# bayesiains/nflows

Hardware: NVIDIA H100
Metric: Flow.log_prob samples/sec, 10-layer RQ-NSF D=784 (higher is better)
Workload: dtype f32

## Files before the change

### nflows_b200/csrc/fused_spline.cuh

```cuda
#pragma once
#include "rq_spline.cuh"
#include "tc_common.cuh"

namespace nfk {
namespace tc {

template <int NB, bool TAILS>
struct FusedCfg {
    static constexpr int M = TAILS ? 3 * NB - 1 : 3 * NB + 1;
    static constexpr int MP = (M + 7) / 8 * 8;
    static constexpr int FPT = BN / (2 * MP);
    static constexpr int TF = 2 * FPT;
    static constexpr int TILE = TF * MP;
    static_assert(FPT >= 1, "unsupported bin count for the fused kernels");
};

struct SplineOut {
    const float* bias;
    const float* x;
    float* y;
    __half* y_hi;
    __half* y_lo;
    const int32_t* t_cols;
    int t_col0;
    float out_scale;
    int64_t ldx, ldy, lds;
    int d_t;
    int inverse;
    float inv_acc_scale;
    SplineParams sp;
};

template <int NB, bool TAILS>
__device__ __forceinline__ int stg_chunk(int r, int c) {
    constexpr int C = FusedCfg<NB, TAILS>::FPT * FusedCfg<NB, TAILS>::MP / 4;
    return c ^ ((0x6530 >> (4 * (r & 3))) & 7) ^ ((C % 8 == 0 && c >= C) ? 4 : 0);
}

template <int NB, bool TAILS, int N>
__device__ __forceinline__ void stage_sums(float* stg, const float (&sum)[N / 2], int wi, int lane) {
#pragma unroll
    for (int j = 0; j < N / 8; ++j)
#pragma unroll
        for (int h = 0; h < 2; ++h) {
            const int r = wi * 16 + (lane >> 2) + 8 * h, c = 2 * j + ((lane & 3) >> 1);
            *reinterpret_cast<float2*>(stg + r * BN + 4 * stg_chunk<NB, TAILS>(r, c) + 2 * (lane & 1)) =
                make_float2(sum[4 * j + 2 * h], sum[4 * j + 2 * h + 1]);
        }
}

template <int NB, bool TAILS>
struct SplineIn {
    float x[FusedCfg<NB, TAILS>::FPT];
    int col[FusedCfg<NB, TAILS>::FPT];
};
template <int NB, bool TAILS>
__device__ __forceinline__ SplineIn<NB, TAILS> spline_inputs(const SplineOut& o, int n, int64_t row, bool row_ok, int fh) {
    constexpr int FPT = FusedCfg<NB, TAILS>::FPT, TF = FusedCfg<NB, TAILS>::TF;
    const int j0 = n * TF + fh * FPT;
    SplineIn<NB, TAILS> in;
#pragma unroll
    for (int f = 0; f < FPT; ++f) {
        const bool ok = row_ok && (j0 + f < o.d_t);
        in.col[f] = !ok ? 0 : (o.t_cols ? __ldg(o.t_cols + j0 + f) : o.t_col0 + j0 + f);
        in.x[f] = ok ? o.x[row * o.ldx + in.col[f]] : 0.0f;
    }
    return in;
}

template <int NB, bool TAILS>
__device__ __forceinline__ void spline_tile(const SplineOut& o, const float* stg, int r, int n, int64_t row, bool row_ok, int fh,
                                            const SplineIn<NB, TAILS>& in, float& lad_row, int& flag) {
    using Cfg = FusedCfg<NB, TAILS>;
    constexpr int MP = Cfg::MP, FPT = Cfg::FPT, TF = Cfg::TF, TILE = Cfg::TILE, C = FPT * MP / 4;
    const int j0 = n * TF + fh * FPT;
    float v[FPT * MP];
    const float* b = o.bias + (int64_t)n * TILE + fh * FPT * MP;
#pragma unroll
    for (int i = 0; i < C; ++i) {
        const float4 s = *reinterpret_cast<const float4*>(stg + r * BN + 4 * stg_chunk<NB, TAILS>(r, fh * C + i));
        const float sv[4] = {s.x, s.y, s.z, s.w};
#pragma unroll
        for (int e = 0; e < 4; ++e) {
            const int c = 4 * i + e;
            v[c] = fmaf(sv[e], o.inv_acc_scale, (j0 + c / MP < o.d_t) ? __ldg(b + c) : 0.0f);
        }
    }
    float yy[FPT], ll[FPT];
    if (o.inverse) rqs_eval_lean<NB, TAILS, true, FPT, MP>(o.sp, in.x, v, yy, ll, flag);
    else rqs_eval_lean<NB, TAILS, false, FPT, MP>(o.sp, in.x, v, yy, ll, flag);
#pragma unroll
    for (int f = 0; f < FPT; ++f) {
        if (!(row_ok && j0 + f < o.d_t)) continue;
        lad_row += ll[f];
        if (o.y_hi) {
            __half hi, lo;
            split_f16(yy[f], o.out_scale, hi, lo, flag);
            o.y_hi[row * o.lds + in.col[f]] = hi;
            o.y_lo[row * o.lds + in.col[f]] = lo;
        } else {
            o.y[row * o.ldy + in.col[f]] = yy[f];
        }
    }
}

}
}
```

### nflows_b200/csrc/nfk_coupling_step_tc.cu

```cuda
#include <stdlib.h>
#include <string.h>

#include "fused_spline.cuh"

namespace nfk {
namespace tc {

constexpr int STEP_MAX_LAYERS = 9;
constexpr int STEP_MAX_HIDDEN = 256;
constexpr int STEP_DRAIN_TRUNK = 4;
constexpr int STEP_DRAIN_FINAL = 8;
constexpr int STEP_SLAB_BYTES = 2 * A_BYTES;
constexpr int STEP_R_BYTES = (STEP_MAX_HIDDEN / BK) * STEP_SLAB_BYTES;
constexpr int STEP_G0_STAGES = STEP_R_BYTES / STAGE_BYTES;
constexpr int STEP_S_OFF = STEP_R_BYTES;
constexpr int STEP_S_WG_BYTES = 32768;
constexpr int STEP_W_OFF = STEP_S_OFF + 2 * STEP_S_WG_BYTES;
constexpr int STEP_W_STAGES = 2;
constexpr int STEP_W_STAGE_BYTES = 2 * B_BYTES;
constexpr int STEP_BAR_OFF = STEP_W_OFF + STEP_W_STAGES * STEP_W_STAGE_BYTES;
constexpr int STEP_LAD_OFF = STEP_BAR_OFF + 256;
constexpr int STEP_SMEM_BYTES = STEP_LAD_OFF + 512 + 1024 ;
static_assert(64 * BN * 4 <= STEP_S_WG_BYTES && 4 * 2 * 64 * 64 <= STEP_S_WG_BYTES, "S");
static_assert(STEP_SMEM_BYTES <= 232448, "coupling-step kernel shared memory");
static_assert(STEP_MAX_HIDDEN / BK <= STEP_DRAIN_FINAL, "the final layer drains once (mma_final)");

constexpr int SL_RELU_OUT = 1;
constexpr int SL_ADD_SKIP = 2;
constexpr int SL_SAVE_SKIP = 4;
constexpr int SL_SPLIT_RELU = 8;

struct StepParams {
    const float* bias_trunk;
    float* skip_buf;
    int H, K0, num_layers;
    int layer_flags[STEP_MAX_LAYERS];
    float acc_scale[STEP_MAX_LAYERS], inv_acc_scale[STEP_MAX_LAYERS];
    float act_scale;
    __half* h_hi;
    __half* h_lo;
    int64_t ldh;
    SplineOut o;
    float* lad_accum;
    int32_t* flags;
    int64_t n_rows;
    int num_m_tiles, num_n_tiles;
};

__device__ __forceinline__ void put_pair(uint8_t* base, int slab_stride, int lo_off, int r, int col, float x0, float x1, float scale,
                                         float& amax) {
    x0 *= scale; x1 *= scale;
    amax = fmaxf(amax, fmaxf(fabsf(x0), fabsf(x1)));
    const __half2 h = __floats2half2_rn(x0, x1);
    const float2 hf = __half22float2(h);
    const __half2 l = __floats2half2_rn(x0 - hf.x, x1 - hf.y);
    const int k = col & 31;
    uint8_t* q = base + (col >> 5) * slab_stride + r * 64 + (((k >> 3) ^ ((r >> 1) & 3)) << 4) + (k & 7) * 2;
    *reinterpret_cast<__half2*>(q) = h;
    *reinterpret_cast<__half2*>(q + lo_off) = l;
}

__device__ __forceinline__ void consumers_sync() { asm volatile("bar.sync 3, 256;" ::: "memory"); }
constexpr int STEP_BAR_TURN = 4;
constexpr int STEP_BAR_LAD = 6;

template <int N, int MH>
__device__ __forceinline__ void mma_final(float (&acc)[MH][N / 2], Ring& r, int num_k, uint32_t a_res, int lane, int turn) {
    int prev = -1;
    for (int j = 0; j < num_k; ++j) {
        mbar_wait(r.full + 8 * r.stage, r.phase);
        if (turn >= 0 && j == num_k - 1) {
            __threadfence_block();
            pair_arrive(turn);
        }
        const uint32_t sw = r.base + r.stage * r.stage_bytes;
        const uint64_t w_hi = make_smem_desc(sw), w_lo = make_smem_desc(sw + B_BYTES);
        wgmma_fence();
#pragma unroll
        for (int m = 0; m < MH; ++m) {
            const uint32_t sa = a_res + (uint32_t)j * STEP_SLAB_BYTES + m * (A_BYTES / 2);
            const uint64_t a_hi = make_smem_desc(sa), a_lo = make_smem_desc(sa + A_BYTES);
#pragma unroll
            for (int kk = 0; kk < BK / 16; ++kk) {
                const uint64_t adv = (uint64_t)(kk * 2);
                wgmma_f16<N>(acc[m], a_lo + adv, w_hi + adv, (j | kk) != 0);
                wgmma_f16<N>(acc[m], a_hi + adv, w_lo + adv, 1);
            }
#pragma unroll
            for (int kk = 0; kk < BK / 16; ++kk) {
                const uint64_t adv = (uint64_t)(kk * 2);
                wgmma_f16<N>(acc[m], a_hi + adv, w_hi + adv, 1);
            }
        }
        wgmma_commit();
        if (prev >= 0) {
            wgmma_wait<1>();
            __syncwarp();
            if (lane == 0) mbar_arrive(r.empty + 8 * prev, MH);
        }
        prev = r.stage;
        r.advance();
    }
    wgmma_wait<0>();
    __syncwarp();
    if (lane == 0) mbar_arrive(r.empty + 8 * prev, MH);
}

template <int NB, bool TAILS>
__global__ void __launch_bounds__(THREADS, 1)
rq_coupling_step_kernel(const __grid_constant__ CUtensorMap map_a_hi, const __grid_constant__ CUtensorMap map_a_lo,
                        const __grid_constant__ CUtensorMap map_w0_hi, const __grid_constant__ CUtensorMap map_w0_lo,
                        const __grid_constant__ CUtensorMap map_wt_hi, const __grid_constant__ CUtensorMap map_wt_lo,
                        const __grid_constant__ CUtensorMap map_wf_hi, const __grid_constant__ CUtensorMap map_wf_lo,
                        const StepParams p) {
    constexpr int TILE = FusedCfg<NB, TAILS>::TILE;
    extern __shared__ uint8_t smem_raw[];
    const uint32_t smem_base = (smem_u32(smem_raw) + 1023u) & ~1023u;
    uint8_t* smem_gen = smem_raw + (smem_base - smem_u32(smem_raw));
    const uint32_t bars = smem_base + STEP_BAR_OFF;
    Ring ring0{smem_base, bars, bars + 8 * STEP_G0_STAGES, STEP_G0_STAGES, (uint32_t)STAGE_BYTES};
    Ring ring1{smem_base + STEP_W_OFF, bars + 64, bars + 64 + 8 * STEP_W_STAGES, STEP_W_STAGES, (uint32_t)STEP_W_STAGE_BYTES};
    const uint32_t bar_rfree = bars + 96;
    const int warp = threadIdx.x >> 5, lane = threadIdx.x & 31;
    const int H = p.H;
    const int num_k0 = (p.K0 + BK - 1) / BK, num_kh = H / BK;
    const int nch = (H + BN - 1) / BN;
    const bool trunk_only = p.h_hi != nullptr;

    if (threadIdx.x == 0) {
        for (int s = 0; s < STEP_G0_STAGES; ++s) { mbar_init(ring0.full + 8 * s, 1); mbar_init(ring0.empty + 8 * s, 8); }
        for (int s = 0; s < STEP_W_STAGES; ++s) { mbar_init(ring1.full + 8 * s, 1); mbar_init(ring1.empty + 8 * s, 8); }
        mbar_init(bar_rfree, 8);
        asm volatile("fence.mbarrier_init.release.cluster;" ::: "memory");
        prefetch_tmap(&map_a_hi); prefetch_tmap(&map_a_lo); prefetch_tmap(&map_w0_hi); prefetch_tmap(&map_w0_lo);
        prefetch_tmap(&map_wt_hi); prefetch_tmap(&map_wt_lo); prefetch_tmap(&map_wf_hi); prefetch_tmap(&map_wf_lo);
    }
    __syncthreads();

    if (warp < 4) {
        asm volatile("setmaxnreg.dec.sync.aligned.u32 40;" ::: "memory");
        if (warp == 0 && elect_one()) {
            uint32_t rphase = 0;
            for (int u = blockIdx.x; u < p.num_m_tiles; u += gridDim.x) {
                if (u != (int)blockIdx.x) { mbar_wait(bar_rfree, rphase); rphase ^= 1; }
                for (int c = 0; c < nch; ++c)
                    for (int ks = 0; ks < num_k0; ++ks) produce_slab(ring0, &map_a_hi, &map_a_lo, &map_w0_hi, &map_w0_lo, ks, u * BM, c * BN);
                for (int l = 1; l < p.num_layers; ++l)
                    for (int c = 0; c < nch; ++c)
                        for (int ks = 0; ks < num_kh; ++ks) produce_w_slab(ring1, &map_wt_hi, &map_wt_lo, ks, (l - 1) * H + c * BN);
                if (!trunk_only)
                    for (int n = 0; n < p.num_n_tiles; ++n)
                        for (int ks = 0; ks < num_kh; ++ks) produce_w_slab(ring1, &map_wf_hi, &map_wf_lo, ks, n * TILE, TILE);
            }
        }
        return;
    }
    asm volatile("setmaxnreg.inc.sync.aligned.u32 232;" ::: "memory");
    const int wg = (warp >> 2) - 1, wi = warp & 3, q = lane & 3;
    const int t = threadIdx.x - 128 * (1 + wg);
    const int r_loc = t >> 1, fh = t & 1;
    uint8_t* R = smem_gen;
    uint8_t* S = smem_gen + STEP_S_OFF + wg * STEP_S_WG_BYTES;
    float* stg = reinterpret_cast<float*>(S);
    float* skip = p.skip_buf + (size_t)blockIdx.x * BM * H;
    int flag = 0;
    for (int u = blockIdx.x; u < p.num_m_tiles; u += gridDim.x) {
        const int64_t m0 = (int64_t)u * BM;
        int rt[2];
        rt[0] = wg * 64 + wi * 16 + (lane >> 2);
        rt[1] = rt[0] + 8;
        for (int l = 0; l < p.num_layers; ++l) {
            const int lf = p.layer_flags[l];
            const bool to_global = trunk_only && l == p.num_layers - 1;
            const float as = p.acc_scale[l], ias = p.inv_acc_scale[l];
            float amax = 0.0f;
            for (int c = 0; c < nch; ++c) {
                const int cb = c * BN + 2 * q;
                float sum[64];
#pragma unroll
                for (int j = 0; j < 16; ++j) {
                    const int col = cb + 8 * j;
#pragma unroll
                    for (int e = 0; e < 2; ++e) {
                        const float b = col < H ? __ldg(p.bias_trunk + l * H + col + e) * as : 0.0f;
#pragma unroll
                        for (int h = 0; h < 2; ++h) {
                            const float sk = ((lf & SL_ADD_SKIP) && col < H) ? skip[rt[h] * H + col + e] : 0.0f;
                            sum[4 * j + 2 * h + e] = fmaf(sk, as, b);
                        }
                    }
                }
                if (l == 0) mma_tile(sum, ring0, num_k0, STEP_DRAIN_TRUNK, wg, lane);
                else mma_tile(sum, ring1, num_kh, STEP_DRAIN_TRUNK, wg, lane, smem_base);
#pragma unroll
                for (int i = 0; i < 64; ++i) {
                    float x = sum[i] * ias;
                    if (lf & SL_RELU_OUT) x = fmaxf(x, 0.0f);
                    sum[i] = x;
                }
                if (lf & SL_SAVE_SKIP) {
#pragma unroll
                    for (int j = 0; j < 16; ++j)
#pragma unroll
                        for (int h = 0; h < 2; ++h)
                            if (cb + 8 * j < H)
                                *reinterpret_cast<float2*>(skip + rt[h] * H + cb + 8 * j) = make_float2(sum[4 * j + 2 * h], sum[4 * j + 2 * h + 1]);
                }
                if (lf & SL_SPLIT_RELU) {
#pragma unroll
                    for (int i = 0; i < 64; ++i) sum[i] = fmaxf(sum[i], 0.0f);
                }
                if (to_global) {
#pragma unroll
                    for (int h = 0; h < 2; ++h) {
                        const int64_t row = m0 + rt[h];
                        if (row >= p.n_rows) continue;
                        float am = 0.0f;
#pragma unroll
                        for (int j = 0; j < 16; ++j) {
                            const int col = cb + 8 * j;
                            if (col >= H) continue;
                            const float x0 = sum[4 * j + 2 * h] * p.act_scale, x1 = sum[4 * j + 2 * h + 1] * p.act_scale;
                            am = fmaxf(am, fmaxf(fabsf(x0), fabsf(x1)));
                            const __half2 hh = __floats2half2_rn(x0, x1);
                            const float2 hf = __half22float2(hh);
                            *reinterpret_cast<__half2*>(p.h_hi + row * p.ldh + col) = hh;
                            *reinterpret_cast<__half2*>(p.h_lo + row * p.ldh + col) = __floats2half2_rn(x0 - hf.x, x1 - hf.y);
                        }
                        if (!(am <= 65000.0f)) flag |= 4;
                    }
                    continue;
                }
                const bool into_r = c == nch - 1;
                if (into_r) {
                    if (l == 0) consumers_sync();
                } else {
                    wg_sync(wg);
                }
#pragma unroll
                for (int h = 0; h < 2; ++h) {
                    float am = 0.0f;
#pragma unroll
                    for (int j = 0; j < 16; ++j) {
                        const int cc = 8 * j + 2 * q;
                        if (c * BN + cc >= H) continue;
                        if (into_r)
                            put_pair(R, STEP_SLAB_BYTES, A_BYTES, rt[h], c * BN + cc, sum[4 * j + 2 * h], sum[4 * j + 2 * h + 1], p.act_scale, am);
                        else
                            put_pair(S, 2 * A_BYTES / 2, A_BYTES / 2, rt[h] - wg * 64, cc, sum[4 * j + 2 * h], sum[4 * j + 2 * h + 1],
                                     p.act_scale, am);
                    }
                    if (m0 + rt[h] < p.n_rows) amax = fmaxf(amax, am);
                }
                if (into_r && nch > 1) {
                    wg_sync(wg);
                    for (int i = t; i < 4 * 2 * 256; i += 128) {
                        const int part = i >> 8, k = i & 255;
                        const uint4 v = reinterpret_cast<const uint4*>(S + part * 4096)[k];
                        reinterpret_cast<uint4*>(R + (part >> 1) * STEP_SLAB_BYTES + (part & 1) * A_BYTES + wg * 4096)[k] = v;
                    }
                }
            }
            if (!(amax <= 65000.0f)) flag |= 4;
            if (!to_global) {
                asm volatile("fence.proxy.async.shared::cta;" ::: "memory");
                wg_sync(wg);
            }
        }
        if (trunk_only) {
            __syncwarp();
            if (lane == 0) mbar_arrive(bar_rfree);
            continue;
        }
        if (p.num_n_tiles == 1) {
            const int64_t srow = m0 + wg * 64 + r_loc;
            const bool row_ok = srow < p.n_rows;
            const SplineIn<NB, TAILS> in = spline_inputs<NB, TAILS>(p.o, 0, srow, row_ok, fh);
            float acc[1][TILE / 2] = {};
            mma_final<TILE, 1>(acc, ring1, num_kh, smem_base + wg * (A_BYTES / 2), lane, -1);
            __syncwarp();
            if (lane == 0) mbar_arrive(bar_rfree);
            stage_sums<NB, TAILS, TILE>(stg, acc[0], wi, lane);
            wg_sync(wg);
            float lad_row = 0.0f;
            spline_tile<NB, TAILS>(p.o, stg, r_loc, 0, srow, row_ok, fh, in, lad_row, flag);
            const float other = __shfl_xor_sync(0xffffffffu, lad_row, 1);
            if (p.lad_accum && fh == 0 && row_ok) p.lad_accum[srow] += lad_row + other;
            continue;
        }
        consumers_sync();
        const int nt = p.num_n_tiles;
        int64_t srow[2];
        bool row_ok[2];
        float lad[2] = {0.0f, 0.0f};
#pragma unroll
        for (int m = 0; m < 2; ++m) {
            srow[m] = m0 + 64 * m + r_loc;
            row_ok[m] = srow[m] < p.n_rows;
        }
        for (int n = 0; n < nt; ++n) {
            if ((n & 1) != wg) {
                for (int ks = 0; ks < num_kh; ++ks) ring1.advance();
                continue;
            }
            SplineIn<NB, TAILS> in[2];
#pragma unroll
            for (int m = 0; m < 2; ++m) in[m] = spline_inputs<NB, TAILS>(p.o, n, srow[m], row_ok[m], fh);
            if (n > 0) pair_wait(STEP_BAR_TURN + wg);
            float acc[2][TILE / 2] = {};
            mma_final<TILE, 2>(acc, ring1, num_kh, smem_base, lane, n + 1 < nt ? STEP_BAR_TURN + (wg ^ 1) : -1);
            if (n + 2 >= nt) {
                __syncwarp();
                if (lane == 0) mbar_arrive(bar_rfree);
            }
#pragma unroll
            for (int m = 0; m < 2; ++m) {
                wg_sync(wg);
                stage_sums<NB, TAILS, TILE>(stg, acc[m], wi, lane);
                wg_sync(wg);
                spline_tile<NB, TAILS>(p.o, stg, r_loc, n, srow[m], row_ok[m], fh, in[m], lad[m], flag);
            }
        }
        float* lad_x = reinterpret_cast<float*>(smem_gen + STEP_LAD_OFF);
#pragma unroll
        for (int m = 0; m < 2; ++m) lad[m] += __shfl_xor_sync(0xffffffffu, lad[m], 1);
        if (wg == 1) {
            if (fh == 0) {
                lad_x[r_loc] = lad[0];
                lad_x[64 + r_loc] = lad[1];
            }
            __threadfence_block();
            pair_arrive(STEP_BAR_LAD);
        } else {
            pair_wait(STEP_BAR_LAD);
            if (p.lad_accum && fh == 0)
#pragma unroll
                for (int m = 0; m < 2; ++m)
                    if (row_ok[m]) p.lad_accum[srow[m]] += lad[m] + lad_x[64 * m + r_loc];
        }
    }
    if (flag && p.flags) atomicOr(p.flags, flag);
}

template <int NB, bool TAILS>
static int launch_step(const NfkCouplingStep* d, StepParams& p, cudaStream_t st) {
    using Cfg = FusedCfg<NB, TAILS>;
    const int H = p.H, L = p.num_layers - 1;
    CUtensorMap ma_hi, ma_lo, mw0_hi, mw0_lo, mwt_hi, mwt_lo, mwf_hi, mwf_lo;
    int rc;
    if ((rc = make_map(&ma_hi, (const __half*)d->a_hi, p.n_rows, p.K0, d->lda, BM))) return rc;
    if ((rc = make_map(&ma_lo, (const __half*)d->a_lo, p.n_rows, p.K0, d->lda, BM))) return rc;
    if ((rc = make_map(&mw0_hi, (const __half*)d->w0_hi, H, p.K0, d->ldw0, BN))) return rc;
    if ((rc = make_map(&mw0_lo, (const __half*)d->w0_lo, H, p.K0, d->ldw0, BN))) return rc;
    mwt_hi = mw0_hi; mwt_lo = mw0_lo;
    if (L > 0) {
        if ((rc = make_map(&mwt_hi, (const __half*)d->wt_hi, (int64_t)L * H, H, d->ldwt, BN))) return rc;
        if ((rc = make_map(&mwt_lo, (const __half*)d->wt_lo, (int64_t)L * H, H, d->ldwt, BN))) return rc;
    }
    mwf_hi = mw0_hi; mwf_lo = mw0_lo;
    p.num_n_tiles = 0;
    if (!p.h_hi) {
        const int packed_rows = p.o.d_t * Cfg::MP;
        if ((rc = make_map(&mwf_hi, (const __half*)d->wp_hi, packed_rows, H, d->ldwp, Cfg::TILE))) return rc;
        if ((rc = make_map(&mwf_lo, (const __half*)d->wp_lo, packed_rows, H, d->ldwp, Cfg::TILE))) return rc;
        p.num_n_tiles = (p.o.d_t + Cfg::TF - 1) / Cfg::TF;
    }
    const int grid = p.num_m_tiles < sm_count() ? p.num_m_tiles : sm_count();
    NFK_REQUIRE(d->workspace_bytes >= (size_t)grid * (size_t)H * BM * 4, "workspace too small: %zu bytes given, %zu needed",
                d->workspace_bytes, (size_t)grid * (size_t)H * BM * 4);
    static DeviceOnce attr_once;
    int attr_dev = 0;
    if (attr_once.pending(&attr_dev)) {
        cudaError_t e = cudaFuncSetAttribute(rq_coupling_step_kernel<NB, TAILS>, cudaFuncAttributeMaxDynamicSharedMemorySize, STEP_SMEM_BYTES);
        if (e != cudaSuccess) return fail(NFK_E_CUDA, "cudaFuncSetAttribute(smem=%d): %s", STEP_SMEM_BYTES, cudaGetErrorString(e));
        attr_once.mark(attr_dev);
    }
    rq_coupling_step_kernel<NB, TAILS><<<grid, THREADS, STEP_SMEM_BYTES, st>>>(ma_hi, ma_lo, mw0_hi, mw0_lo, mwt_hi, mwt_lo, mwf_hi,
                                                                             mwf_lo, p);
    return check_launch("rq_coupling_step_kernel");
}

}
}

using namespace nfk;

extern "C" int nfk_rq_coupling_step_supported(int32_t num_bins, int32_t linear_tails, int32_t hidden_features, int32_t in_features,
                                              int32_t num_square_layers) {
    const bool bins_ok = (num_bins == 8 || num_bins == 10 || num_bins == 4 || num_bins == 16);
    return (bins_ok && hidden_features >= 32 && hidden_features <= tc::STEP_MAX_HIDDEN && hidden_features % 32 == 0 && in_features >= 8 &&
            in_features % 8 == 0 && num_square_layers >= 0 && num_square_layers < tc::STEP_MAX_LAYERS) ? 1 : 0;
}

extern "C" size_t nfk_rq_coupling_step_workspace_bytes(int32_t hidden_features) {
    return (size_t)tc::sm_count() * (size_t)hidden_features * tc::BM * 4;
}

extern "C" int nfk_rq_coupling_step_f16x3(const NfkCouplingStep* d, void* stream) {
    NFK_REQUIRE(d, "NULL descriptor");
    NFK_REQUIRE(d->n_rows >= 0 && d->hidden_features >= 1 && d->in_features >= 1, "bad sizes");
    if (d->n_rows == 0) return NFK_OK;
    const bool trunk_only = d->h_hi != nullptr;
    const int nb = trunk_only && !d->spline ? 8 : (d->spline ? d->spline->num_bins : 0);
    const int lt = trunk_only && !d->spline ? 1 : (d->spline ? d->spline->linear_tails : 0);
    NFK_REQUIRE(trunk_only || d->spline, "spline descriptor missing");
    NFK_REQUIRE(nfk_rq_coupling_step_supported(nb, lt, d->hidden_features, d->in_features, d->num_square_layers),
                "coupling-step kernel does not take num_bins=%d hidden=%d in_features=%d square layers=%d", nb, d->hidden_features,
                d->in_features, d->num_square_layers);
    NFK_REQUIRE(d->a_hi && d->a_lo && d->w0_hi && d->w0_lo && d->bias_trunk && d->layer_flags && d->workspace, "NULL pointer");
    NFK_REQUIRE(d->num_square_layers == 0 || (d->wt_hi && d->wt_lo && d->wt_exps), "square-layer weights missing");
    NFK_REQUIRE(d->lda % 8 == 0 && d->ldw0 % 8 == 0 && (d->num_square_layers == 0 || d->ldwt % 8 == 0), "row pitches must be multiples of 8");
    NFK_REQUIRE(aligned16(d->a_hi) && aligned16(d->a_lo) && aligned16(d->w0_hi) && aligned16(d->w0_lo) && aligned16(d->bias_trunk) &&
                    aligned16(d->workspace) && (d->num_square_layers == 0 || (aligned16(d->wt_hi) && aligned16(d->wt_lo))),
                "operands must be 16-byte aligned");
    NFK_REQUIRE(d->n_rows < (1ll << 31), "n_rows too large for one launch");
    const int H = d->hidden_features, L = d->num_square_layers;
    for (int l = 0; l <= L; ++l) {
        const int lf = d->layer_flags[l];
        const int e = l == 0 ? d->a_exp + d->w0_exp : d->act_exp + d->wt_exps[l - 1];
        NFK_REQUIRE(!((lf & tc::SL_ADD_SKIP) && (lf & tc::SL_RELU_OUT)), "layer %d: skip add after a relu output is not supported", l);
        NFK_REQUIRE(e >= -60 && e <= 60, "scale exponent out of range");
    }
    if (trunk_only) {
        NFK_REQUIRE(d->h_lo && d->ldh % 8 == 0 && aligned16(d->h_hi) && aligned16(d->h_lo), "bad trunk output pair");
    } else {
        NFK_REQUIRE(d->wp_hi && d->wp_lo && d->bias_packed && d->x && d->d_t >= 1, "NULL pointer");
        NFK_REQUIRE((d->y != nullptr) != (d->y_hi != nullptr), "give either y (fp32 outputs) or y_hi / y_lo (their fp16 split pair)");
        NFK_REQUIRE((d->y_hi == nullptr) == (d->y_lo == nullptr) && d->y_exp >= -60 && d->y_exp <= 60, "bad pair output");
        NFK_REQUIRE(d->t_cols || d->t_col0 >= 0, "t_cols is NULL and t_col0 is negative");
        NFK_REQUIRE(aligned16(d->bias_packed) && aligned16(d->wp_hi) && aligned16(d->wp_lo) && d->ldwp % 8 == 0,
                    "packed final layer must be 16-byte aligned");
        NFK_REQUIRE(d->act_exp + d->wp_exp >= -60 && d->act_exp + d->wp_exp <= 60, "scale exponent out of range");
    }
    tc::StepParams p;
    memset(&p, 0, sizeof(p));
    p.bias_trunk = d->bias_trunk; p.skip_buf = (float*)d->workspace; p.H = H; p.K0 = d->in_features;
    p.num_layers = 1 + L; p.act_scale = ldexpf(1.0f, d->act_exp);
    for (int l = 0; l <= L; ++l) {
        const int e = l == 0 ? d->a_exp + d->w0_exp : d->act_exp + d->wt_exps[l - 1];
        p.layer_flags[l] = d->layer_flags[l];
        p.acc_scale[l] = ldexpf(1.0f, e);
        p.inv_acc_scale[l] = ldexpf(1.0f, -e);
    }
    p.flags = d->flags; p.n_rows = d->n_rows;
    p.num_m_tiles = (int)((d->n_rows + tc::BM - 1) / tc::BM);
    cudaStream_t st = (cudaStream_t)stream;
    if (trunk_only) {
        p.h_hi = (__half*)d->h_hi; p.h_lo = (__half*)d->h_lo; p.ldh = d->ldh;
        return tc::launch_step<8, true>(d, p, st);
    }
    int rc = make_spline_params(d->spline, &p.o.sp);
    if (rc) return rc;
    p.o.bias = d->bias_packed; p.o.x = d->x; p.o.y = d->y; p.o.y_hi = (__half*)d->y_hi; p.o.y_lo = (__half*)d->y_lo;
    p.o.t_cols = d->t_cols; p.o.t_col0 = d->t_col0; p.o.out_scale = ldexpf(1.0f, d->y_exp); p.o.ldx = d->ldx; p.o.ldy = d->ldy;
    p.o.lds = d->lds; p.o.d_t = d->d_t; p.o.inverse = d->inverse; p.o.inv_acc_scale = ldexpf(1.0f, -(d->act_exp + d->wp_exp));
    p.lad_accum = d->lad_accum;
    const bool tails = d->spline->linear_tails != 0;
#define NFK_STEP(NB) return tails ? tc::launch_step<NB, true>(d, p, st) : tc::launch_step<NB, false>(d, p, st)
    switch (d->spline->num_bins) {
        case 4: NFK_STEP(4);
        case 8: NFK_STEP(8);
        case 10: NFK_STEP(10);
        case 16: NFK_STEP(16);
    }
#undef NFK_STEP
    return fail(NFK_E_UNSUPPORTED, "num_bins=%d has no coupling-step kernel instance", d->spline->num_bins);
}
```

### nflows_b200/csrc/tc_common.cuh

```cuda
#pragma once
#include <cuda.h>
#include <cuda_fp16.h>

#include "nfk_common.cuh"

namespace nfk {
namespace tc {

constexpr int BM = 128;
constexpr int BN = 128;
constexpr int BK = 32;
constexpr int THREADS = 384;
constexpr int A_BYTES = BM * BK * 2;
constexpr int B_BYTES = BN * BK * 2;
constexpr int STAGE_BYTES = 2 * A_BYTES + 2 * B_BYTES;
constexpr int ROW_BYTES = BK * 2;
constexpr int DRAIN_SLABS_LINEAR = 2;
constexpr int DRAIN_SLABS_FUSED = 4;

__device__ __forceinline__ uint32_t smem_u32(const void* p) { return (uint32_t)__cvta_generic_to_shared(p); }

__device__ __forceinline__ void mbar_init(uint32_t bar, uint32_t count) {
    asm volatile("mbarrier.init.shared::cta.b64 [%0], %1;" ::"r"(bar), "r"(count) : "memory");
}
__device__ __forceinline__ void mbar_expect_tx(uint32_t bar, uint32_t bytes) {
    asm volatile("mbarrier.arrive.expect_tx.shared::cta.b64 _, [%0], %1;" ::"r"(bar), "r"(bytes) : "memory");
}
__device__ __forceinline__ void mbar_arrive(uint32_t bar) {
    asm volatile("mbarrier.arrive.shared::cta.b64 _, [%0];" ::"r"(bar) : "memory");
}
__device__ __forceinline__ void mbar_arrive(uint32_t bar, uint32_t count) {
    asm volatile("mbarrier.arrive.shared::cta.b64 _, [%0], %1;" ::"r"(bar), "r"(count) : "memory");
}
__device__ __forceinline__ void mbar_wait(uint32_t bar, uint32_t parity) {
    asm volatile(
        "{\n"
        ".reg .pred p;\n"
        "WAIT_%=:\n"
        "mbarrier.try_wait.parity.shared::cta.b64 p, [%0], %1;\n"
        "@p bra DONE_%=;\n"
        "bra WAIT_%=;\n"
        "DONE_%=:\n"
        "}\n" ::"r"(bar),
        "r"(parity)
        : "memory");
}
__device__ __forceinline__ void tma_load_2d(uint32_t dst, const CUtensorMap* map, uint32_t bar, int c0, int c1) {
    asm volatile(
        "cp.async.bulk.tensor.2d.shared::cluster.global.mbarrier::complete_tx::bytes [%0], [%1, {%3, %4}], [%2];" ::"r"(dst),
        "l"(reinterpret_cast<uint64_t>(map)), "r"(bar), "r"(c0), "r"(c1)
        : "memory");
}
__device__ __forceinline__ void prefetch_tmap(const CUtensorMap* map) {
    asm volatile("prefetch.tensormap [%0];" ::"l"(reinterpret_cast<uint64_t>(map)) : "memory");
}
__device__ __forceinline__ bool elect_one() {
    uint32_t pred = 0;
    asm volatile(
        "{\n"
        ".reg .pred P1;\n"
        "elect.sync _|P1, 0xffffffff;\n"
        "selp.u32 %0, 1, 0, P1;\n"
        "}\n"
        : "+r"(pred));
    return pred != 0;
}
__device__ __forceinline__ void wg_sync(int wg) { asm volatile("bar.sync %0, 128;" ::"r"(1 + wg) : "memory"); }
__device__ __forceinline__ void pair_arrive(int id) { asm volatile("bar.arrive %0, 256;" ::"r"(id) : "memory"); }
__device__ __forceinline__ void pair_wait(int id) { asm volatile("bar.sync %0, 256;" ::"r"(id) : "memory"); }

__device__ __forceinline__ void wgmma_fence() { asm volatile("wgmma.fence.sync.aligned;" ::: "memory"); }
__device__ __forceinline__ void wgmma_commit() { asm volatile("wgmma.commit_group.sync.aligned;" ::: "memory"); }
template <int N>
__device__ __forceinline__ void wgmma_wait() { asm volatile("wgmma.wait_group.sync.aligned %0;" ::"n"(N) : "memory"); }

template <int N>
__device__ __forceinline__ void wgmma_f16(float (&d)[N / 2], uint64_t adesc, uint64_t bdesc, uint32_t accumulate);
template <>
__device__ __forceinline__ void wgmma_f16<128>(float (&d)[64], uint64_t adesc, uint64_t bdesc, uint32_t accumulate) {
    asm volatile(
        "{\n"
        ".reg .pred p;\n"
        "setp.ne.b32 p, %66, 0;\n"
        "wgmma.mma_async.sync.aligned.m64n128k16.f32.f16.f16 {"
        "%0, %1, %2, %3, %4, %5, %6, %7, %8, %9, %10, %11, %12, %13, %14, %15, "
        "%16, %17, %18, %19, %20, %21, %22, %23, %24, %25, %26, %27, %28, %29, %30, %31, "
        "%32, %33, %34, %35, %36, %37, %38, %39, %40, %41, %42, %43, %44, %45, %46, %47, "
        "%48, %49, %50, %51, %52, %53, %54, %55, %56, %57, %58, %59, %60, %61, %62, %63}, "
        "%64, %65, p, 1, 1, 0, 0;\n"
        "}\n"
        : "+f"(d[0]), "+f"(d[1]), "+f"(d[2]), "+f"(d[3]), "+f"(d[4]), "+f"(d[5]), "+f"(d[6]), "+f"(d[7]),
          "+f"(d[8]), "+f"(d[9]), "+f"(d[10]), "+f"(d[11]), "+f"(d[12]), "+f"(d[13]), "+f"(d[14]), "+f"(d[15]),
          "+f"(d[16]), "+f"(d[17]), "+f"(d[18]), "+f"(d[19]), "+f"(d[20]), "+f"(d[21]), "+f"(d[22]), "+f"(d[23]),
          "+f"(d[24]), "+f"(d[25]), "+f"(d[26]), "+f"(d[27]), "+f"(d[28]), "+f"(d[29]), "+f"(d[30]), "+f"(d[31]),
          "+f"(d[32]), "+f"(d[33]), "+f"(d[34]), "+f"(d[35]), "+f"(d[36]), "+f"(d[37]), "+f"(d[38]), "+f"(d[39]),
          "+f"(d[40]), "+f"(d[41]), "+f"(d[42]), "+f"(d[43]), "+f"(d[44]), "+f"(d[45]), "+f"(d[46]), "+f"(d[47]),
          "+f"(d[48]), "+f"(d[49]), "+f"(d[50]), "+f"(d[51]), "+f"(d[52]), "+f"(d[53]), "+f"(d[54]), "+f"(d[55]),
          "+f"(d[56]), "+f"(d[57]), "+f"(d[58]), "+f"(d[59]), "+f"(d[60]), "+f"(d[61]), "+f"(d[62]), "+f"(d[63])
        : "l"(adesc), "l"(bdesc), "r"(accumulate)
        : "memory");
}

template <>
__device__ __forceinline__ void wgmma_f16<112>(float (&d)[56], uint64_t adesc, uint64_t bdesc, uint32_t accumulate) {
    asm volatile(
        "{\n"
        ".reg .pred p;\n"
        "setp.ne.b32 p, %58, 0;\n"
        "wgmma.mma_async.sync.aligned.m64n112k16.f32.f16.f16 {"
        "%0, %1, %2, %3, %4, %5, %6, %7, %8, %9, %10, %11, %12, %13, %14, %15, "
        "%16, %17, %18, %19, %20, %21, %22, %23, %24, %25, %26, %27, %28, %29, %30, %31, "
        "%32, %33, %34, %35, %36, %37, %38, %39, %40, %41, %42, %43, %44, %45, %46, %47, "
        "%48, %49, %50, %51, %52, %53, %54, %55}, "
        "%56, %57, p, 1, 1, 0, 0;\n"
        "}\n"
        : "+f"(d[0]), "+f"(d[1]), "+f"(d[2]), "+f"(d[3]), "+f"(d[4]), "+f"(d[5]), "+f"(d[6]), "+f"(d[7]),
          "+f"(d[8]), "+f"(d[9]), "+f"(d[10]), "+f"(d[11]), "+f"(d[12]), "+f"(d[13]), "+f"(d[14]), "+f"(d[15]),
          "+f"(d[16]), "+f"(d[17]), "+f"(d[18]), "+f"(d[19]), "+f"(d[20]), "+f"(d[21]), "+f"(d[22]), "+f"(d[23]),
          "+f"(d[24]), "+f"(d[25]), "+f"(d[26]), "+f"(d[27]), "+f"(d[28]), "+f"(d[29]), "+f"(d[30]), "+f"(d[31]),
          "+f"(d[32]), "+f"(d[33]), "+f"(d[34]), "+f"(d[35]), "+f"(d[36]), "+f"(d[37]), "+f"(d[38]), "+f"(d[39]),
          "+f"(d[40]), "+f"(d[41]), "+f"(d[42]), "+f"(d[43]), "+f"(d[44]), "+f"(d[45]), "+f"(d[46]), "+f"(d[47]),
          "+f"(d[48]), "+f"(d[49]), "+f"(d[50]), "+f"(d[51]), "+f"(d[52]), "+f"(d[53]), "+f"(d[54]), "+f"(d[55])
        : "l"(adesc), "l"(bdesc), "r"(accumulate)
        : "memory");
}

template <>
__device__ __forceinline__ void wgmma_f16<96>(float (&d)[48], uint64_t adesc, uint64_t bdesc, uint32_t accumulate) {
    asm volatile(
        "{\n"
        ".reg .pred p;\n"
        "setp.ne.b32 p, %50, 0;\n"
        "wgmma.mma_async.sync.aligned.m64n96k16.f32.f16.f16 {"
        "%0, %1, %2, %3, %4, %5, %6, %7, %8, %9, %10, %11, %12, %13, %14, %15, "
        "%16, %17, %18, %19, %20, %21, %22, %23, %24, %25, %26, %27, %28, %29, %30, %31, "
        "%32, %33, %34, %35, %36, %37, %38, %39, %40, %41, %42, %43, %44, %45, %46, %47}, "
        "%48, %49, p, 1, 1, 0, 0;\n"
        "}\n"
        : "+f"(d[0]), "+f"(d[1]), "+f"(d[2]), "+f"(d[3]), "+f"(d[4]), "+f"(d[5]), "+f"(d[6]), "+f"(d[7]),
          "+f"(d[8]), "+f"(d[9]), "+f"(d[10]), "+f"(d[11]), "+f"(d[12]), "+f"(d[13]), "+f"(d[14]), "+f"(d[15]),
          "+f"(d[16]), "+f"(d[17]), "+f"(d[18]), "+f"(d[19]), "+f"(d[20]), "+f"(d[21]), "+f"(d[22]), "+f"(d[23]),
          "+f"(d[24]), "+f"(d[25]), "+f"(d[26]), "+f"(d[27]), "+f"(d[28]), "+f"(d[29]), "+f"(d[30]), "+f"(d[31]),
          "+f"(d[32]), "+f"(d[33]), "+f"(d[34]), "+f"(d[35]), "+f"(d[36]), "+f"(d[37]), "+f"(d[38]), "+f"(d[39]),
          "+f"(d[40]), "+f"(d[41]), "+f"(d[42]), "+f"(d[43]), "+f"(d[44]), "+f"(d[45]), "+f"(d[46]), "+f"(d[47])
        : "l"(adesc), "l"(bdesc), "r"(accumulate)
        : "memory");
}

static_assert(ROW_BYTES == 64, "descriptors assume 64-byte K-slab rows");
__device__ __forceinline__ uint64_t make_smem_desc(uint32_t saddr) {
    return (uint64_t)((saddr & 0x3FFFFu) >> 4) | (1ull << 16) | ((uint64_t)((8 * ROW_BYTES) >> 4) << 32) | (2ull << 62);
}

struct Ring {
    uint32_t base, full, empty;
    int stages;
    uint32_t stage_bytes;
    int stage = 0;
    uint32_t phase = 0;
    __device__ __forceinline__ void advance() {
        if (++stage == stages) { stage = 0; phase ^= 1; }
    }
};

__device__ __forceinline__ void produce_slab(Ring& r, const CUtensorMap* a_hi, const CUtensorMap* a_lo, const CUtensorMap* w_hi,
                                             const CUtensorMap* w_lo, int ks, int m0, int n0) {
    mbar_wait(r.empty + 8 * r.stage, r.phase ^ 1);
    const uint32_t full = r.full + 8 * r.stage;
    const uint32_t sa = r.base + r.stage * r.stage_bytes;
    mbar_expect_tx(full, STAGE_BYTES);
    tma_load_2d(sa, a_hi, full, ks * BK, m0);
    tma_load_2d(sa + A_BYTES, a_lo, full, ks * BK, m0);
    tma_load_2d(sa + 2 * A_BYTES, w_hi, full, ks * BK, n0);
    tma_load_2d(sa + 2 * A_BYTES + B_BYTES, w_lo, full, ks * BK, n0);
    r.advance();
}

__device__ __forceinline__ void produce_w_slab(Ring& r, const CUtensorMap* w_hi, const CUtensorMap* w_lo, int ks, int n0, int rows = BN) {
    mbar_wait(r.empty + 8 * r.stage, r.phase ^ 1);
    const uint32_t full = r.full + 8 * r.stage;
    const uint32_t sw = r.base + r.stage * r.stage_bytes;
    mbar_expect_tx(full, 2 * rows * ROW_BYTES);
    tma_load_2d(sw, w_hi, full, ks * BK, n0);
    tma_load_2d(sw + B_BYTES, w_lo, full, ks * BK, n0);
    r.advance();
}

__device__ __forceinline__ void mma_tile(float (&sum)[64], Ring& r, int num_k, int drain, int wg, int lane, uint32_t a_res = 0) {
    float acc[64];
    for (int g0 = 0; g0 < num_k; g0 += drain) {
        const int slabs = min(drain, num_k - g0);
        int prev = -1;
        for (int j = 0; j < slabs; ++j) {
            mbar_wait(r.full + 8 * r.stage, r.phase);
            const uint32_t ss = r.base + r.stage * r.stage_bytes;
            const uint32_t sa = a_res ? a_res + (uint32_t)(g0 + j) * 2 * A_BYTES : ss;
            const uint32_t sw = a_res ? ss : ss + 2 * A_BYTES;
            const uint64_t a_hi = make_smem_desc(sa + wg * (A_BYTES / 2)), a_lo = make_smem_desc(sa + A_BYTES + wg * (A_BYTES / 2));
            const uint64_t w_hi = make_smem_desc(sw), w_lo = make_smem_desc(sw + B_BYTES);
            wgmma_fence();
#pragma unroll
            for (int kk = 0; kk < BK / 16; ++kk) {
                const uint64_t adv = (uint64_t)(kk * 2);
                wgmma_f16<BN>(acc, a_lo + adv, w_hi + adv, (j | kk) != 0);
                wgmma_f16<BN>(acc, a_hi + adv, w_lo + adv, 1);
            }
#pragma unroll
            for (int kk = 0; kk < BK / 16; ++kk) {
                const uint64_t adv = (uint64_t)(kk * 2);
                wgmma_f16<BN>(acc, a_hi + adv, w_hi + adv, 1);
            }
            wgmma_commit();
            if (prev >= 0) {
                wgmma_wait<1>();
                __syncwarp();
                if (lane == 0) mbar_arrive(r.empty + 8 * prev);
            }
            prev = r.stage;
            r.advance();
        }
        wgmma_wait<0>();
        __syncwarp();
        if (lane == 0) mbar_arrive(r.empty + 8 * prev);
#pragma unroll
        for (int i = 0; i < 64; ++i) sum[i] = __fadd_rn(sum[i], acc[i]);
    }
}

__device__ __forceinline__ void split_f16(float v, float scale, __half& hi, __half& lo, int& flag) {
    const float s = v * scale;
    if (!(fabsf(s) <= 65000.0f)) flag |= 4;
    hi = __float2half_rn(s);
    lo = __float2half_rn(s - __half2float(hi));
}

int make_map(CUtensorMap* map, const __half* base, int64_t rows, int K, int64_t ld, int box_rows);

}
}
```

Baseline: 1.720 million.

## Give the final coupling layer its own deeper weight ring and compact staging buffers

```diff
diff --git a/nflows_b200/csrc/fused_spline.cuh b/nflows_b200/csrc/fused_spline.cuh
--- a/nflows_b200/csrc/fused_spline.cuh
+++ b/nflows_b200/csrc/fused_spline.cuh
@@ -12,6 +12,7 @@
     static constexpr int FPT = BN / (2 * MP);
     static constexpr int TF = 2 * FPT;
     static constexpr int TILE = TF * MP;
+    static constexpr int SP = (TILE / 4 + 7) / 8 * 8 * 4;
     static_assert(FPT >= 1, "unsupported bin count for the fused kernels");
 };
 
@@ -37,14 +38,15 @@
     return c ^ ((0x6530 >> (4 * (r & 3))) & 7) ^ ((C % 8 == 0 && c >= C) ? 4 : 0);
 }
 
-template <int NB, bool TAILS, int N>
+template <int NB, bool TAILS, int N, int SP = BN>
 __device__ __forceinline__ void stage_sums(float* stg, const float (&sum)[N / 2], int wi, int lane) {
+    static_assert(SP % 32 == 0 && N <= SP, "staging row stride");
 #pragma unroll
     for (int j = 0; j < N / 8; ++j)
 #pragma unroll
         for (int h = 0; h < 2; ++h) {
             const int r = wi * 16 + (lane >> 2) + 8 * h, c = 2 * j + ((lane & 3) >> 1);
-            *reinterpret_cast<float2*>(stg + r * BN + 4 * stg_chunk<NB, TAILS>(r, c) + 2 * (lane & 1)) =
+            *reinterpret_cast<float2*>(stg + r * SP + 4 * stg_chunk<NB, TAILS>(r, c) + 2 * (lane & 1)) =
                 make_float2(sum[4 * j + 2 * h], sum[4 * j + 2 * h + 1]);
         }
 }
@@ -68,7 +70,7 @@
     return in;
 }
 
-template <int NB, bool TAILS>
+template <int NB, bool TAILS, int SP = BN>
 __device__ __forceinline__ void spline_tile(const SplineOut& o, const float* stg, int r, int n, int64_t row, bool row_ok, int fh,
                                             const SplineIn<NB, TAILS>& in, float& lad_row, int& flag) {
     using Cfg = FusedCfg<NB, TAILS>;
@@ -78,7 +80,7 @@
     const float* b = o.bias + (int64_t)n * TILE + fh * FPT * MP;
 #pragma unroll
     for (int i = 0; i < C; ++i) {
-        const float4 s = *reinterpret_cast<const float4*>(stg + r * BN + 4 * stg_chunk<NB, TAILS>(r, fh * C + i));
+        const float4 s = *reinterpret_cast<const float4*>(stg + r * SP + 4 * stg_chunk<NB, TAILS>(r, fh * C + i));
         const float sv[4] = {s.x, s.y, s.z, s.w};
 #pragma unroll
         for (int e = 0; e < 4; ++e) {
diff --git a/nflows_b200/csrc/nfk_coupling_step_tc.cu b/nflows_b200/csrc/nfk_coupling_step_tc.cu
--- a/nflows_b200/csrc/nfk_coupling_step_tc.cu
+++ b/nflows_b200/csrc/nfk_coupling_step_tc.cu
@@ -13,17 +13,34 @@
 constexpr int STEP_SLAB_BYTES = 2 * A_BYTES;
 constexpr int STEP_R_BYTES = (STEP_MAX_HIDDEN / BK) * STEP_SLAB_BYTES;
 constexpr int STEP_G0_STAGES = STEP_R_BYTES / STAGE_BYTES;
-constexpr int STEP_S_OFF = STEP_R_BYTES;
 constexpr int STEP_S_WG_BYTES = 32768;
-constexpr int STEP_W_OFF = STEP_S_OFF + 2 * STEP_S_WG_BYTES;
+constexpr int STEP_S0_OFF = STEP_R_BYTES;
+constexpr int STEP_W_OFF = STEP_S0_OFF + STEP_S_WG_BYTES;
 constexpr int STEP_W_STAGES = 2;
 constexpr int STEP_W_STAGE_BYTES = 2 * B_BYTES;
-constexpr int STEP_BAR_OFF = STEP_W_OFF + STEP_W_STAGES * STEP_W_STAGE_BYTES;
+constexpr int STEP_S1_OFF = STEP_W_OFF + STEP_W_STAGES * STEP_W_STAGE_BYTES;
+constexpr int STEP_BAR_OFF = STEP_S1_OFF + STEP_S_WG_BYTES;
 constexpr int STEP_LAD_OFF = STEP_BAR_OFF + 256;
 constexpr int STEP_SMEM_BYTES = STEP_LAD_OFF + 512 + 1024 ;
-static_assert(64 * BN * 4 <= STEP_S_WG_BYTES && 4 * 2 * 64 * 64 <= STEP_S_WG_BYTES, "S");
+static_assert(4 * 2 * 64 * 64 <= STEP_S_WG_BYTES, "S0, S1");
 static_assert(STEP_SMEM_BYTES <= 232448, "coupling-step kernel shared memory");
 static_assert(STEP_MAX_HIDDEN / BK <= STEP_DRAIN_FINAL, "the final layer drains once (mma_final)");
+
+template <int NB, bool TAILS>
+struct StepFinal {
+    static constexpr int TILE = FusedCfg<NB, TAILS>::TILE, SP = FusedCfg<NB, TAILS>::SP;
+    static constexpr int STG_BYTES = 64 * SP * 4;
+    static constexpr int STG1_OFF = STEP_BAR_OFF - STG_BYTES;
+    static constexpr int LO_OFF = TILE * ROW_BYTES;
+    static constexpr int STAGE_BYTES = 2 * LO_OFF;
+    static constexpr int RING_OFF = STEP_S0_OFF + STG_BYTES;
+    static constexpr int STAGES = (STG1_OFF - RING_OFF) / STAGE_BYTES;
+    static constexpr int MAX_STAGES = 4;
+    static_assert(STG_BYTES <= STEP_S_WG_BYTES, "staged sums inside the warpgroup's own first-chunk pair");
+    static_assert(STAGES >= STEP_W_STAGES && STAGES <= MAX_STAGES, "final-layer ring depth");
+    static_assert(TILE != 96 || STAGES == 4, "TILE = 96: 4 stages");
+    static_assert(LO_OFF % 1024 == 0 && RING_OFF % 1024 == 0 && STAGE_BYTES % 1024 == 0, "SWIZZLE_64B stage alignment");
+};
 
 constexpr int SL_RELU_OUT = 1;
 constexpr int SL_ADD_SKIP = 2;
@@ -74,7 +91,7 @@
             pair_arrive(turn);
         }
         const uint32_t sw = r.base + r.stage * r.stage_bytes;
-        const uint64_t w_hi = make_smem_desc(sw), w_lo = make_smem_desc(sw + B_BYTES);
+        const uint64_t w_hi = make_smem_desc(sw), w_lo = make_smem_desc(sw + N * ROW_BYTES);
         wgmma_fence();
 #pragma unroll
         for (int m = 0; m < MH; ++m) {
@@ -113,7 +130,8 @@
                         const __grid_constant__ CUtensorMap map_wt_hi, const __grid_constant__ CUtensorMap map_wt_lo,
                         const __grid_constant__ CUtensorMap map_wf_hi, const __grid_constant__ CUtensorMap map_wf_lo,
                         const StepParams p) {
-    constexpr int TILE = FusedCfg<NB, TAILS>::TILE;
+    using F = StepFinal<NB, TAILS>;
+    constexpr int TILE = F::TILE;
     extern __shared__ uint8_t smem_raw[];
     const uint32_t smem_base = (smem_u32(smem_raw) + 1023u) & ~1023u;
     uint8_t* smem_gen = smem_raw + (smem_base - smem_u32(smem_raw));
@@ -121,6 +139,9 @@
     Ring ring0{smem_base, bars, bars + 8 * STEP_G0_STAGES, STEP_G0_STAGES, (uint32_t)STAGE_BYTES};
     Ring ring1{smem_base + STEP_W_OFF, bars + 64, bars + 64 + 8 * STEP_W_STAGES, STEP_W_STAGES, (uint32_t)STEP_W_STAGE_BYTES};
     const uint32_t bar_rfree = bars + 96;
+    const uint32_t bar_ffree = bars + 104;
+    Ring ringf{smem_base + F::RING_OFF, bars + 112, bars + 112 + 8 * F::MAX_STAGES, F::STAGES, (uint32_t)F::STAGE_BYTES};
+    static_assert(112 + 16 * F::MAX_STAGES <= 256, "barriers");
     const int warp = threadIdx.x >> 5, lane = threadIdx.x & 31;
     const int H = p.H;
     const int num_k0 = (p.K0 + BK - 1) / BK, num_kh = H / BK;
@@ -130,7 +151,9 @@
     if (threadIdx.x == 0) {
         for (int s = 0; s < STEP_G0_STAGES; ++s) { mbar_init(ring0.full + 8 * s, 1); mbar_init(ring0.empty + 8 * s, 8); }
         for (int s = 0; s < STEP_W_STAGES; ++s) { mbar_init(ring1.full + 8 * s, 1); mbar_init(ring1.empty + 8 * s, 8); }
+        for (int s = 0; s < F::STAGES; ++s) { mbar_init(ringf.full + 8 * s, 1); mbar_init(ringf.empty + 8 * s, 8); }
         mbar_init(bar_rfree, 8);
+        mbar_init(bar_ffree, 8);
         asm volatile("fence.mbarrier_init.release.cluster;" ::: "memory");
         prefetch_tmap(&map_a_hi); prefetch_tmap(&map_a_lo); prefetch_tmap(&map_w0_hi); prefetch_tmap(&map_w0_lo);
         prefetch_tmap(&map_wt_hi); prefetch_tmap(&map_wt_lo); prefetch_tmap(&map_wf_hi); prefetch_tmap(&map_wf_lo);
@@ -140,7 +163,7 @@
     if (warp < 4) {
         asm volatile("setmaxnreg.dec.sync.aligned.u32 40;" ::: "memory");
         if (warp == 0 && elect_one()) {
-            uint32_t rphase = 0;
+            uint32_t rphase = 0, fphase = 0;
             for (int u = blockIdx.x; u < p.num_m_tiles; u += gridDim.x) {
                 if (u != (int)blockIdx.x) { mbar_wait(bar_rfree, rphase); rphase ^= 1; }
                 for (int c = 0; c < nch; ++c)
@@ -148,9 +171,11 @@
                 for (int l = 1; l < p.num_layers; ++l)
                     for (int c = 0; c < nch; ++c)
                         for (int ks = 0; ks < num_kh; ++ks) produce_w_slab(ring1, &map_wt_hi, &map_wt_lo, ks, (l - 1) * H + c * BN);
-                if (!trunk_only)
-                    for (int n = 0; n < p.num_n_tiles; ++n)
-                        for (int ks = 0; ks < num_kh; ++ks) produce_w_slab(ring1, &map_wf_hi, &map_wf_lo, ks, n * TILE, TILE);
+                if (trunk_only) continue;
+                mbar_wait(bar_ffree, fphase);
+                fphase ^= 1;
+                for (int n = 0; n < p.num_n_tiles; ++n)
+                    for (int ks = 0; ks < num_kh; ++ks) produce_w_slab(ringf, &map_wf_hi, &map_wf_lo, ks, n * TILE, TILE, F::LO_OFF);
             }
         }
         return;
@@ -160,8 +185,7 @@
     const int t = threadIdx.x - 128 * (1 + wg);
     const int r_loc = t >> 1, fh = t & 1;
     uint8_t* R = smem_gen;
-    uint8_t* S = smem_gen + STEP_S_OFF + wg * STEP_S_WG_BYTES;
-    float* stg = reinterpret_cast<float*>(S);
+    uint8_t* S = smem_gen + STEP_S0_OFF + wg * (STEP_S1_OFF - STEP_S0_OFF);
     float* skip = p.skip_buf + (size_t)blockIdx.x * BM * H;
     int flag = 0;
     for (int u = blockIdx.x; u < p.num_m_tiles; u += gridDim.x) {
@@ -169,6 +193,11 @@
         int rt[2];
         rt[0] = wg * 64 + wi * 16 + (lane >> 2);
         rt[1] = rt[0] + 8;
+        {
+            const int slabs = (u - (int)blockIdx.x) / (int)gridDim.x * (p.num_layers - 1) * nch * num_kh;
+            ring1.stage = slabs % STEP_W_STAGES;
+            ring1.phase = (slabs / STEP_W_STAGES) & 1;
+        }
         for (int l = 0; l < p.num_layers; ++l) {
             const int lf = p.layer_flags[l];
             const bool to_global = trunk_only && l == p.num_layers - 1;
@@ -267,23 +296,25 @@
                 wg_sync(wg);
             }
         }
+        __syncwarp();
         if (trunk_only) {
-            __syncwarp();
             if (lane == 0) mbar_arrive(bar_rfree);
             continue;
         }
+        if (lane == 0) mbar_arrive(bar_ffree);
+        float* stg = reinterpret_cast<float*>(smem_gen + STEP_S0_OFF + wg * (F::STG1_OFF - STEP_S0_OFF));
         if (p.num_n_tiles == 1) {
             const int64_t srow = m0 + wg * 64 + r_loc;
             const bool row_ok = srow < p.n_rows;
             const SplineIn<NB, TAILS> in = spline_inputs<NB, TAILS>(p.o, 0, srow, row_ok, fh);
             float acc[1][TILE / 2] = {};
-            mma_final<TILE, 1>(acc, ring1, num_kh, smem_base + wg * (A_BYTES / 2), lane, -1);
+            mma_final<TILE, 1>(acc, ringf, num_kh, smem_base + wg * (A_BYTES / 2), lane, -1);
             __syncwarp();
             if (lane == 0) mbar_arrive(bar_rfree);
-            stage_sums<NB, TAILS, TILE>(stg, acc[0], wi, lane);
+            stage_sums<NB, TAILS, TILE, F::SP>(stg, acc[0], wi, lane);
             wg_sync(wg);
             float lad_row = 0.0f;
-            spline_tile<NB, TAILS>(p.o, stg, r_loc, 0, srow, row_ok, fh, in, lad_row, flag);
+            spline_tile<NB, TAILS, F::SP>(p.o, stg, r_loc, 0, srow, row_ok, fh, in, lad_row, flag);
             const float other = __shfl_xor_sync(0xffffffffu, lad_row, 1);
             if (p.lad_accum && fh == 0 && row_ok) p.lad_accum[srow] += lad_row + other;
             continue;
@@ -300,7 +331,7 @@
         }
         for (int n = 0; n < nt; ++n) {
             if ((n & 1) != wg) {
-                for (int ks = 0; ks < num_kh; ++ks) ring1.advance();
+                for (int ks = 0; ks < num_kh; ++ks) ringf.advance();
                 continue;
             }
             SplineIn<NB, TAILS> in[2];
@@ -308,7 +339,7 @@
             for (int m = 0; m < 2; ++m) in[m] = spline_inputs<NB, TAILS>(p.o, n, srow[m], row_ok[m], fh);
             if (n > 0) pair_wait(STEP_BAR_TURN + wg);
             float acc[2][TILE / 2] = {};
-            mma_final<TILE, 2>(acc, ring1, num_kh, smem_base, lane, n + 1 < nt ? STEP_BAR_TURN + (wg ^ 1) : -1);
+            mma_final<TILE, 2>(acc, ringf, num_kh, smem_base, lane, n + 1 < nt ? STEP_BAR_TURN + (wg ^ 1) : -1);
             if (n + 2 >= nt) {
                 __syncwarp();
                 if (lane == 0) mbar_arrive(bar_rfree);
@@ -316,9 +347,9 @@
 #pragma unroll
             for (int m = 0; m < 2; ++m) {
                 wg_sync(wg);
-                stage_sums<NB, TAILS, TILE>(stg, acc[m], wi, lane);
+                stage_sums<NB, TAILS, TILE, F::SP>(stg, acc[m], wi, lane);
                 wg_sync(wg);
-                spline_tile<NB, TAILS>(p.o, stg, r_loc, n, srow[m], row_ok[m], fh, in[m], lad[m], flag);
+                spline_tile<NB, TAILS, F::SP>(p.o, stg, r_loc, n, srow[m], row_ok[m], fh, in[m], lad[m], flag);
             }
         }
         float* lad_x = reinterpret_cast<float*>(smem_gen + STEP_LAD_OFF);
diff --git a/nflows_b200/csrc/tc_common.cuh b/nflows_b200/csrc/tc_common.cuh
--- a/nflows_b200/csrc/tc_common.cuh
+++ b/nflows_b200/csrc/tc_common.cuh
@@ -176,13 +176,14 @@
     r.advance();
 }
 
-__device__ __forceinline__ void produce_w_slab(Ring& r, const CUtensorMap* w_hi, const CUtensorMap* w_lo, int ks, int n0, int rows = BN) {
+__device__ __forceinline__ void produce_w_slab(Ring& r, const CUtensorMap* w_hi, const CUtensorMap* w_lo, int ks, int n0, int rows = BN,
+                                               uint32_t lo_off = B_BYTES) {
     mbar_wait(r.empty + 8 * r.stage, r.phase ^ 1);
     const uint32_t full = r.full + 8 * r.stage;
     const uint32_t sw = r.base + r.stage * r.stage_bytes;
     mbar_expect_tx(full, 2 * rows * ROW_BYTES);
     tma_load_2d(sw, w_hi, full, ks * BK, n0);
-    tma_load_2d(sw + B_BYTES, w_lo, full, ks * BK, n0);
+    tma_load_2d(sw + lo_off, w_lo, full, ks * BK, n0);
     r.advance();
 }
 
```

After: 1.876 million, median of 6. 1.09x the previous value.
